# PoTaTo-Mika/fish-speech

Hardware: AMD Instinct MI355X
Metric: audio-sec/wall-sec (RTF) + p50 first-sample latency, S2-Pro 4B @1/2/4/8 GPU (higher is better)
Workload: dtype bf16; 1 GPU; BASELINE config 2 per GPU: one utterance = 64-token prompt + 216 Dual-AR frames (top_k 30, top_p 0.8, temp 0.8) + codec decode [1,10,216] -> 442368 samples; global_batch=1, frames=216, prompt_len=64, first_chunk_frames=1, vocoder_chunks=first_chunk_frames, then growing 4x, vocoder=serial, parallelism=dp1

## Files before the change

fish-speech_amd/csrc/fm_attn.hip:

```cpp
#include "fm_kernels.h"
#include "fm_runtime.h"
#include "fm_attn_dev.h"
#include "fm_frag.h"

template <typename T>
__device__ __forceinline__ void head_prep(const T* src, int hd, bool norm, const T* nw, float eps,
                                          const float* tab, bool do_rope, float (&x0)[2],
                                          float (&x1)[2], int& np, int lane) {
    const int half = hd >> 1;
    np = 0;
    for (int p = lane; p < half; p += 64, ++np) {
        x0[np] = ld(src, 2 * p);
        x1[np] = ld(src, 2 * p + 1);
    }
    if (norm) {
        float ss = 0.f;
        for (int i = 0; i < np; ++i) ss += x0[i] * x0[i] + x1[i] * x1[i];
        ss = wave_sum(ss);
        const float rs = 1.0f / sqrtf(ss / (float)hd + eps);
        for (int i = 0; i < np; ++i) {
            const int p = lane + 64 * i;
            x0[i] = rnd<T>((x0[i] * rs) * ld(nw, 2 * p));
            x1[i] = rnd<T>((x1[i] * rs) * ld(nw, 2 * p + 1));
        }
// ... 491 lines not shown
}
template <typename T> __device__ __forceinline__ typename Frag<T>::f frag_f32(const float* v) {
    typename Frag<T>::f f;
    if constexpr (sizeof(T) == 2) {
#pragma unroll
        for (int i = 0; i < 4; ++i) f[i] = hi_pair(v[2 * i], v[2 * i + 1]);
    } else {
#pragma unroll
        for (int i = 0; i < 4; ++i) {
            f.lo[i] = v[i];
            f.hi[i] = v[4 + i];
        }
    }
    return f;
}
template <typename T, int HD, int NW>
__global__ __launch_bounds__(NW * 64) void attn_fd_kernel(AttnDecArgs<T> a) {
    static_assert(HD % 32 == 0 && HD <= 128, "head_dim a multiple of 32 up to 128");
    constexpr int NT = NW * 64, FD_TILE = 16 * NW;
    constexpr int VL = 8 * (int)sizeof(T) / 16;
    constexpr int half = HD / 2;
    __shared__ __attribute__((aligned(16))) float q_s[FD_GM][HD];
    __shared__ __attribute__((aligned(16))) float kv_new[2][HD];
    __shared__ __attribute__((aligned(16))) float wml[NW][FD_GM][2];
    constexpr int OG = NW > 4 ? 1 : 4;
    __shared__ __attribute__((aligned(16))) float ored[NW][OG][FD_GM][HD];
    __shared__ int flag;
    unsigned long long tz[7] = {0, 0, 0, 0, 0, 0, 0};
    DBG_TS(tz, 0)
    const int lane = threadIdx.x & 63, wave = threadIdx.x >> 6;
    const int l16 = lane & 15, qq = lane >> 4;
    const int r = blockIdx.x, kvh = blockIdx.y, sp = blockIdx.z;
    const int g = a.nh / a.nkv, nitem = g + 2;
    const int slot = a.row_slot[r];
    const int pos = a.row_pos[r];
    constexpr int NI = (2 + FD_GM + NW - 1) / NW;
    float x0[NI], x1[NI];
#pragma unroll
    for (int i = 0; i < NI; ++i) {
        const int it = wave + NW * i;
        const int row = it < g ? kvh * g + it : (it == g ? a.nh + kvh : a.nh + a.nkv + kvh);
        const bool ok = it < nitem && lane < half;
        float v0, v1;
        raw_pair<T>(a.qkv, a.ldqkv, a.qslab, a.qslab_kp, gridDim.x, a.qbias, r,
                    (size_t)(it < nitem ? row : 0) * HD + 2 * (lane < half ? lane : 0), v0, v1);
        x0[i] = ok ? v0 : 0.f;
        x1[i] = ok ? v1 : 0.f;
    }
    const int npos = pos + 1;
    int nsp = min((int)gridDim.z, (npos + a.cap - 1) / a.cap);
    const int chunk = ((npos + nsp - 1) / nsp + 15) & ~15;
    nsp = (npos + chunk - 1) / chunk;
    if (sp >= nsp) return;
    const int j0 = sp * chunk, jend = min(j0 + chunk, npos);
    const bool owner = jend == npos;
    const size_t base = (size_t)slot * a.slot_stride + a.layer_off + (size_t)kvh * a.S * HD;
    T* kc = a.kc + base;
    T* vc = a.vc + base;
    const int vd = 8 * l16 < HD ? 8 * l16 : HD - 8;
    using F = Frag<T>;
    constexpr int NKS = HD / 32;
    typename F::f kb[NKS];
    u32x4_t vb[4][VL];
    auto issue = [&](int jb) {
        const int jk = min(jb + 16 * wave + l16, jend - 1);
// ... 23 lines not shown
                x0[i] = rnd<T>((x0[i] * rs) * ld(nw, 2 * lane));
                x1[i] = rnd<T>((x1[i] * rs) * ld(nw, 2 * lane + 1));
            }
        }
        if (lane < half) {
            float y0 = x0[i], y1 = x1[i];
            if (isq || isk) {
                const float c = rcs.x, sn = rcs.y;
                y0 = rnd<T>(x0[i] * c - x1[i] * sn);
                y1 = rnd<T>(x1[i] * c + x0[i] * sn);
            }
            if (isq) {
                q_s[it][2 * lane] = y0;
                q_s[it][2 * lane + 1] = y1;
                if (a.qdbg && sp == 0) {
                    float* qdp = a.qdbg + ((size_t)r * a.nh + kvh * g + it) * HD;
                    qdp[2 * lane] = y0;
                    qdp[2 * lane + 1] = y1;
                }
            } else {
                kv_new[isk ? 0 : 1][2 * lane] = y0;
                kv_new[isk ? 0 : 1][2 * lane + 1] = y1;
                T* dst = (isk ? kc : vc) + (size_t)pos * HD;
                st(dst, 2 * lane, y0);
                st(dst, 2 * lane + 1, y1);
            }
        }
    }
    lds_barrier();
    DBG_TS(tz, 1)
    const int qh = l16 >> 2;
    const bool qrow = (l16 & 3) == 0 && qh < g;
    typename F::f qa[NKS];
#pragma unroll
    for (int ks = 0; ks < NKS; ++ks) {
        float qv[8];
#pragma unroll
        for (int e = 0; e < 8; ++e) qv[e] = qrow ? q_s[qh][32 * ks + 8 * qq + e] : 0.f;
        qa[ks] = frag_f32<T>(qv);
    }
    __shared__ __attribute__((aligned(16))) float p_s[NW][16][FD_GM];
    float m_run = -INFINITY, l_run = 0.f, o[FD_GM][8];
#pragma unroll
    for (int h = 0; h < FD_GM; ++h)
#pragma unroll
        for (int e = 0; e < 8; ++e) o[h][e] = 0.f;
    const int npass = (jend - j0 + FD_TILE - 1) / FD_TILE;
    for (int pa = 0; pa < npass; ++pa) {
        const int jb = j0 + pa * FD_TILE;
        const int jk = jb + 16 * wave + l16;
        if (owner && jk == pos) {
#pragma unroll
            for (int ks = 0; ks < NKS; ++ks) kb[ks] = frag_f32<T>(&kv_new[0][32 * ks + 8 * qq]);
        }
        f32x4_t sc = {0.f, 0.f, 0.f, 0.f};
#pragma unroll
        for (int ks = 0; ks < NKS; ++ks) sc = F::mma(qa[ks], kb[ks], sc);
        float vf[4][8];
#pragma unroll
// ... 9 lines not shown
        if (owner) {
#pragma unroll
            for (int it = 0; it < 4; ++it)
                if (min(jb + 16 * wave + 4 * it + qq, jend - 1) == pos)
#pragma unroll
                    for (int e = 0; e < 8; ++e) vf[it][e] = kv_new[1][vd + e];
        }
        const bool kval = jk < jend && qq < g;
        {
            const float sv = kval ? sc[0] * a.scale : -INFINITY;
            const float mnew = fmaxf(m_run, row_max16(sv));
            const float alpha = mnew == -INFINITY ? 1.f : expf(m_run - mnew);
            const float p = kval ? expf(sv - mnew) : 0.f;
            m_run = mnew;
            l_run = l_run * alpha + p;
            p_s[wave][l16][qq] = p;
#pragma unroll
            for (int h = 0; h < FD_GM; ++h) {
                if (h >= g) break;
                const float ah = __int_as_float(__builtin_amdgcn_readlane(__float_as_int(alpha), 16 * h));
#pragma unroll
                for (int e = 0; e < 8; ++e) o[h][e] *= ah;
            }
        }
        __builtin_amdgcn_wave_barrier();
#pragma unroll
        for (int it = 0; it < 4; ++it) {
            const f32x4_t pv = *reinterpret_cast<const f32x4_t*>(&p_s[wave][4 * it + qq][0]);
#pragma unroll
            for (int h = 0; h < FD_GM; ++h) {
                if (h >= g) break;
#pragma unroll
                for (int e = 0; e < 8; ++e) o[h][e] += pv[h] * vf[it][e];
            }
        }
        __builtin_amdgcn_wave_barrier();
    }
    DBG_TS(tz, 2)
    const float lrow = row_sum16(l_run);
    if (l16 == 0 && qq < g) {
        wml[wave][qq][0] = m_run;
        wml[wave][qq][1] = lrow;
    }
#pragma unroll
    for (int h = 0; h < FD_GM; ++h) {
        if (h >= g) break;
        if constexpr (OG == 1) {
#pragma unroll
            for (int e = 0; e < 8; ++e) o[h][e] = sum_rows4(o[h][e], lane);
        }
        if (8 * l16 < HD && (OG == 4 || qq == 0)) {
            f32x4_t* dst = reinterpret_cast<f32x4_t*>(&ored[wave][OG == 4 ? qq : 0][h][8 * l16]);
            dst[0] = (f32x4_t){o[h][0], o[h][1], o[h][2], o[h][3]};
            dst[1] = (f32x4_t){o[h][4], o[h][5], o[h][6], o[h][7]};
        }
    }
    DBG_TS(tz, 5)
    lds_barrier();
    DBG_TS(tz, 3)
    const bool single = nsp == 1;
// ... 1 lines not shown
        const int h = idx / HD, e = idx - h * HD;
        float M = wml[0][h][0];
#pragma unroll
        for (int w = 1; w < NW; ++w) M = fmaxf(M, wml[w][h][0]);
        float L = 0.f, O = 0.f;
#pragma unroll
        for (int w = 0; w < NW; ++w) {
            const float sc = expf(wml[w][h][0] - M);
            L += sc * wml[w][h][1];
            if constexpr (OG == 4)
                O += sc * ((ored[w][0][h][e] + ored[w][1][h][e]) + (ored[w][2][h][e] + ored[w][3][h][e]));
            else
                O += sc * ored[w][0][h][e];
        }
        if (single) {
            st(a.out + (size_t)r * a.nh * HD + (size_t)(kvh * g + h) * HD, e, O / L);
        } else {
            float* pp = a.part + (((size_t)r * a.nh + (size_t)kvh * g + h) * a.maxsplit + sp) * (HD + 2);
            __hip_atomic_store(pp + 2 + e, O, __ATOMIC_RELAXED, __HIP_MEMORY_SCOPE_AGENT);
            if (e == 0) {
                __hip_atomic_store(pp, M, __ATOMIC_RELAXED, __HIP_MEMORY_SCOPE_AGENT);
                __hip_atomic_store(pp + 1, L, __ATOMIC_RELAXED, __HIP_MEMORY_SCOPE_AGENT);
            }
        }
    }
    if (a.dbg && threadIdx.x == 0) {
        tz[4] = __builtin_amdgcn_s_memrealtime();
        dbg_record(a.dbg, 0xFFFC, (unsigned)(nsp << 16 | (jend - j0)), tz);
    }
    if (single) return;
    asm volatile("s_waitcnt vmcnt(0)" ::: "memory");
    __syncthreads();
    if (threadIdx.x == 0) {
        const int t = __hip_atomic_fetch_add(a.cnt + (size_t)r * a.nkv + kvh, 1, __ATOMIC_RELAXED,
                                             __HIP_MEMORY_SCOPE_AGENT);
        flag = t == nsp - 1;
        if (t == nsp - 1) __hip_atomic_store(a.cnt + (size_t)r * a.nkv + kvh, 0, __ATOMIC_RELAXED, __HIP_MEMORY_SCOPE_AGENT);
    }
    __syncthreads();
    if (!flag) return;
    DBG_TS(tz, 5)
    constexpr int PP = FD_GM * HD * 8 / NT;
    const int q = l16, grp = threadIdx.x >> 4;
    const int k0 = grp * PP, h = k0 / half, e0 = 2 * (k0 - h * half);
    if (h >= g) return;
    const int qc = q < nsp ? q : nsp - 1;
    const unsigned long long* pp = reinterpret_cast<const unsigned long long*>(
        a.part + (((size_t)r * a.nh + (size_t)kvh * g + h) * a.maxsplit + qc) * (HD + 2));
    const unsigned long long ml = __hip_atomic_load(pp, __ATOMIC_RELAXED, __HIP_MEMORY_SCOPE_AGENT);
    unsigned long long ov[PP];
#pragma unroll
    for (int j = 0; j < PP; ++j) ov[j] = __hip_atomic_load(pp + 1 + e0 / 2 + j, __ATOMIC_RELAXED, __HIP_MEMORY_SCOPE_AGENT);
    const float mq = q < nsp ? __uint_as_float((unsigned)ml) : -INFINITY;
    const float lq = __uint_as_float((unsigned)(ml >> 32));
    float M = mq;
#pragma unroll
    for (int m = 1; m < 16; m <<= 1) M = fmaxf(M, __shfl_xor(M, m));
    const float w = q < nsp ? expf(mq - M) : 0.f;
    float L = w * lq;
#pragma unroll
    for (int m = 1; m < 16; m <<= 1) L += __shfl_xor(L, m);
    T* out = a.out + (size_t)r * a.nh * HD + (size_t)(kvh * g + h) * HD + e0;
#pragma unroll
    for (int j = 0; j < PP; ++j) {
        float o0 = w * __uint_as_float((unsigned)ov[j]), o1 = w * __uint_as_float((unsigned)(ov[j] >> 32));
#pragma unroll
        for (int m = 1; m < 16; m <<= 1) {
            o0 += __shfl_xor(o0, m);
            o1 += __shfl_xor(o1, m);
        }
        if (q == (j & 15)) {
            st(out, 2 * j, o0 / L);
            st(out, 2 * j + 1, o1 / L);
        }
    }
    if (a.dbg && threadIdx.x == 0) {
        tz[6] = __builtin_amdgcn_s_memrealtime();
// ... 750 lines not shown
                                      : ((code >= 0 && code < a.cb) ? code : 0);
    }
    record();
}

template <typename T> void launch_attn_decode2(hipStream_t s, const AttnDecArgs<T>& a, int R) {
    dim3 g1(R, a.nkv, a.maxsplit);
    static bool attr = false;
    if (!attr) {
        (void)hipFuncSetAttribute(reinterpret_cast<const void*>(&attn_decode2_kernel<T>),
                                  hipFuncAttributeMaxDynamicSharedMemorySize, 160 * 1024);
        attr = true;
    }
    attn_decode2_kernel<T><<<g1, 512, attn2_lds_bytes(a.hd, a.nh / a.nkv, a.cap, sizeof(T)), s>>>(a);
}
template <typename T> void launch_attn_fd(hipStream_t s, const AttnDecArgs<T>& a0, int R) {
    FMCHECK(attn_fd_ok(a0.hd, a0.nh / a0.nkv), "attn_fd: head_dim 32, 64 or 128 and at most 4 q heads per kv head");
    FMCHECK(a0.cap >= 16 && a0.cnt && a0.part && a0.out, "attn_fd: min split >= 16, tickets, partials and output set");
    AttnDecArgs<T> a = a0;
    a.maxsplit = std::min(FD_NSP, FM_CEIL(a.S, a.cap));
    const dim3 grid(R, a.nkv, a.maxsplit);
    if (a.nwb == 16) {
        switch (a.hd) {
            case 32: attn_fd_kernel<T, 32, 16><<<grid, 1024, 0, s>>>(a); break;
            case 64: attn_fd_kernel<T, 64, 16><<<grid, 1024, 0, s>>>(a); break;
            default: attn_fd_kernel<T, 128, 16><<<grid, 1024, 0, s>>>(a); break;
        }
        return;
    }
    if (a.nwb == 8) {
        switch (a.hd) {
            case 32: attn_fd_kernel<T, 32, 8><<<grid, 512, 0, s>>>(a); break;
            case 64: attn_fd_kernel<T, 64, 8><<<grid, 512, 0, s>>>(a); break;
            default: attn_fd_kernel<T, 128, 8><<<grid, 512, 0, s>>>(a); break;
        }
        return;
    }
    switch (a.hd) {
        case 32: attn_fd_kernel<T, 32, 4><<<grid, 256, 0, s>>>(a); break;
        case 64: attn_fd_kernel<T, 64, 4><<<grid, 256, 0, s>>>(a); break;
        default: attn_fd_kernel<T, 128, 4><<<grid, 256, 0, s>>>(a); break;
    }
}
template <typename T> void launch_attn_decode3(hipStream_t s, const AttnDecArgs<T>& a0, int R) {
    FMCHECK(a0.hd % 32 == 0 && a0.hd <= 128 && a0.nh % a0.nkv == 0 && a0.nh / a0.nkv <= 6,
            "attn_dec3: hd a multiple of 32 up to 128, at most 6 q heads per kv head");
    AttnDecArgs<T> a = a0;
    a.maxsplit = FM_CEIL(a.S, ATT3_CH);
    attn_dec3_kernel<T><<<dim3(R, a.nkv, a.maxsplit), 256, 0, s>>>(a);
}
template <typename T> void launch_fast_attn2(hipStream_t s, const FastFusedArgs<T>& a, int R) {
    fast_attn2_kernel<T><<<dim3(R, a.nh), 64, 0, s>>>(a);
}
template <typename T> void launch_fast_attn_fused(hipStream_t s, const FastFusedArgs<T>& a, int R) {
    dim3 g(R, a.nkv);
    const size_t lds = (size_t)2 * a.S * a.hd * 4 + (size_t)4 * a.hd * 4 + 4 * 64 * 4;
    fast_attn_fused_kernel<T><<<g, 256, lds, s>>>(a);
// ... 33 lines not shown
```

fish-speech_amd/csrc/fm_kernels.h:

```cpp
#pragma once
#include <algorithm>
#include "fm_common.h"
#include "fm_tune_table.h"

enum { EPI_STORE = 0, EPI_RESID = 1, EPI_SWIGLU = 2, EPI_F32 = 3 };

template <typename T> void launch_swiglu_i8(hipStream_t s, const T* t, int ldt, T* act, int lda, int inter, int R);
template <typename T> void launch_pack(hipStream_t s, const T* src, int N, int K, T* dst);
template <typename T> void launch_quant_rows(hipStream_t s, T* w, int N, int K, int8_t* q, T* scale);
template <typename T> void launch_i8_to(hipStream_t s, const int8_t* q, int64_t n, T* dst);
void launch_pack_q8(hipStream_t s, const int8_t* src, int N, int K, int8_t* dst);
void launch_pack_q8s(hipStream_t s, const int8_t* src, int N, int K, int8_t* dst);
void launch_quant4(hipStream_t s, bf16_t* w, int N, int K, int gs, uint8_t* q, uint32_t* sz);
void launch_pack_q4(hipStream_t s, const uint8_t* q, int N, int K, uint8_t* dst);
void launch_pack_q4_rows(hipStream_t s, const uint8_t* q, int N, int K, uint32_t* dst);
void launch_pack_sz4(hipStream_t s, const uint32_t* sz, int N, int K, int gs, uint32_t* dst);
void launch_pack_q4s(hipStream_t s, const uint8_t* q, int N, int K, uint32_t* dst);

template <typename T> struct LinearArgs {
    const T* W;
    const T* W2;
    const T* bias;
    const T* X;
    int ldx, R, N, K;
// ... 359 lines not shown
    const T* qn;
    const T* kn;
    const float* rope;
    T* kc;
    T* vc;
    size_t slot_stride, layer_off;
    int S, maxsplit;
    float scale;
    float* part;
    int cap;
    int* cnt;
    T* out;
    unsigned long long* dbg;
    float* qdbg = nullptr;
    int nwb = 4;
    const float* qslab = nullptr;
    int qslab_kp = 1;
    const T* qbias = nullptr;
};
template <typename T> void launch_attn_decode2(hipStream_t s, const AttnDecArgs<T>& a, int R);
inline size_t attn2_lds_bytes(int hd, int g, int cap, size_t esz) {
    return (size_t)cap * (hd + 8) * esz + (size_t)cap * hd * esz + (size_t)g * hd * 4 + (size_t)g * cap * 4 +
           16 + 8 * (size_t)g * 4;
}
inline int attn2_cap(int hd, int g, size_t esz) {
    long budget = 150L * 1024 - 16 - 8L * g * 4 - (long)g * hd * 4;
    long per = (long)(2 * hd + 8) * (long)esz + 4L * g;
    long c = budget / per;
    c = c > 256 ? 256 : c;
    return (int)(c & ~15L);
// ... 14 lines not shown
```

fish-speech_amd/csrc/fm_llm_frame.cpp:

```cpp
#include <math.h>

#include <algorithm>
#include <array>

#include "fm_codec.h"
#include "fm_llm_model.h"

template <typename T> struct Run {
    typedef T type_t;
    fm_llm* m;
    hipStream_t s;
    int64_t E;
    bool rows_distinct_slots = false, bs_frame = false, x_ss = false;
    struct BsPending {
        bool on = false;
        const float* slab = nullptr;
        int kparts = 0, d = 0, R = 0;
        void* res = nullptr;
        void* out = nullptr;
        const void* sc = nullptr;
    } pend;
    std::vector<std::array<int, 2>> segs;
    void set_pending(const float* slab, int kparts, int d, int R, void* res, void* out, const void* sc) {
        pend = BsPending{true, slab, kparts, d, R, res, out, sc};
// ... 159 lines not shown
        const int64_t bytes = step_wbytes(a.Wq4s ? 2 : (a.Wq8s ? 1 : 0), N, K, E) + (int64_t)R * K * E +
                              (int64_t)R * N * (epi == EPI_F32 ? 4 : E);
        const double flops = 2.0 * R * N * K;
        hipStream_t st = s;
        auto go = [st, a, epi] { launch_linear<T>(st, a, epi); };
        launch(cls, bytes, flops, go);
    }

    void attn_slow(const AttnDecArgs<T>& aa, int R) { attn_slow_on(s, aa, R); }
    static void attn_slow_on(hipStream_t s, const AttnDecArgs<T>& aa, int R) {
        const AttnSlowPlan p = attn_slow_plan(R, aa.hd, aa.nh / aa.nkv, aa.cap);
        if (p.kernel == 3) {
            AttnDecArgs<T> b = aa;
            b.cap = p.cap;
            b.nwb = p.nwb;
            launch_attn_fd<T>(s, b, R);
        } else if (p.kernel == 2)
            launch_attn_decode3<T>(s, aa, R);
        else
            launch_attn_decode2<T>(s, aa, R);
    }
    bool bs_use(int R, bool) const {
        return (fm_tuning().bstream || m->compact) && bs_frame && R > GEMV_MAX_ROWS && R <= 32 && m->bsA;
    }
    struct BsExtra {
        int pro = PRO_PLAIN;
        const float* ss_in = nullptr;
        const void* nw = nullptr;
        const void* res = nullptr;
        void* res_out = nullptr;
// ... 1281 lines not shown
```

fish-speech_amd/csrc/fm_llm_model.h:

```cpp
#pragma once
#include <hip/hip_runtime.h>

#include <algorithm>

#include "fm_kernels.h"
#include "fm_runtime.h"

static constexpr int PREFILL_CHUNK = 1024;
static constexpr int ATTN_PIECE = 256;
static constexpr int ATTN_SPLIT = 64;
static constexpr int GEMV_MAX_ROWS = 8;
static constexpr int KSB_MAX = 8;

inline int attn2_frame_cap(int hd, int g, size_t esz, bool batched) {
    const int cap = attn2_cap(hd, g, esz), knob = batched ? fm_tuning().attn_cap_batched : fm_tuning().attn_cap;
    return knob ? std::min(cap, knob) : cap;
}
struct AttnSlowPlan {
    int kernel, nwb, cap;
};
inline AttnSlowPlan attn_slow_plan(int R, int hd, int g, int cap0) {
    const FmTuning& tu = fm_tuning();
    if (tu.attn_fd && attn_fd_ok(hd, g)) {
        AttnSlowPlan p{3, 4, std::max(16, R > GEMV_MAX_ROWS ? tu.fd_min_batched : tu.fd_min)};
        if (R <= GEMV_MAX_ROWS && tu.fd_nw > 4) {
            p.nwb = tu.fd_nw;
            p.cap = std::max(16, tu.fd_min16);
        } else if (R > GEMV_MAX_ROWS && tu.fd_nw_batched > 4) {
            p.nwb = tu.fd_nw_batched;
        }
        return p;
    }
    if (tu.attn3 && R > GEMV_MAX_ROWS && hd % 32 == 0 && hd <= 128 && g <= 6) return {2, 4, cap0};
    return {0, 4, cap0};
}
static constexpr int BS_KPARTS = 8;

inline int pick_ksb(int N, int K, int R, size_t esz) {
    const int nb = (N + 15) / 16;
// ... 174 lines not shown
```

fish-speech_amd/csrc/fm_llm_weights.cpp:

```cpp
#include "fm_llm_model.h"

void add_t(fm_llm* m, const std::string& n, int64_t rows, int64_t cols) {
    DTensor t;
    t.rows = rows;
    t.cols = cols;
    t.numel = rows * cols;
    m->w[n] = t;
}
static void add_stack(fm_llm* m, const std::string& pre, const StackDims& s) {
    for (int i = 0; i < s.n_layer; ++i) {
        std::string p = pre + std::to_string(i) + ".";
        add_t(m, p + "attention.wqkv.weight", s.nqkv(), s.dim);
        if (s.qkv_bias) add_t(m, p + "attention.wqkv.bias", 1, s.nqkv());
        add_t(m, p + "attention.wo.weight", s.dim, s.nq());
        if (s.o_bias) add_t(m, p + "attention.wo.bias", 1, s.dim);
        if (s.qk_norm) {
            add_t(m, p + "attention.q_norm.weight", 1, s.hd);
            add_t(m, p + "attention.k_norm.weight", 1, s.hd);
        }
        add_t(m, p + "feed_forward.w1.weight", s.inter, s.dim);
        add_t(m, p + "feed_forward.w3.weight", s.inter, s.dim);
        add_t(m, p + "feed_forward.w2.weight", s.dim, s.inter);
        add_t(m, p + "ffn_norm.weight", 1, s.dim);
        add_t(m, p + "attention_norm.weight", 1, s.dim);
// ... 432 lines not shown
    m->xl = m->dalloc((size_t)n * dmax * E);
    m->plast = m->dalloc((size_t)n * dmax * E);
    m->xnl = m->dalloc((size_t)n * dmax * E);
    m->fx = m->dalloc((size_t)std::max(n, 2) * dmax * E);
    m->fh = m->dalloc((size_t)std::max(n, 2) * dmax * E);
    m->fxn = m->dalloc((size_t)n * dmax * E);
    m->x2 = m->dalloc((size_t)std::min(n, GEMV_MAX_ROWS) * dmax * E);
    m->fx2 = m->dalloc((size_t)std::max(std::min(n, GEMV_MAX_ROWS), 2) * dmax * E);
    m->chain_cnt = (unsigned*)m->dalloc(GEMV_CHAIN_WORDS * sizeof(unsigned));
    m->chain_err = (int*)m->dalloc(16 * sizeof(int));
    HIPCHK(hipHostMalloc((void**)&m->h_chain_err, 16 * sizeof(int), hipHostMallocDefault));
    m->h_chain_err[0] = 0;
    m->maxsplit = FM_CEIL(m->S, ATTN_SPLIT);
    const int Rpart = std::max(m->max_slots, ATTN_PIECE);
    m->part = (float*)m->dalloc((size_t)Rpart * d.nh * std::max(m->maxsplit, FM_CEIL(m->S, 16)) * (d.hd + 2) * 4, false);
    m->attn_cnt = (int*)m->dalloc((size_t)R * d.nkv * sizeof(int));
    m->ssX = (float*)m->dalloc((size_t)(dmax / 16) * std::min(n, 32) * 4);
    m->ssH = (float*)m->dalloc((size_t)(dmax / 16) * std::min(n, 32) * 4);
    {
        const int maxn = std::max({m->Nhead, 2 * c.intermediate_size, 2 * c.fast_intermediate_size, qkvmax, dmax, m->cb});
        m->tickets = (int*)m->dalloc((size_t)(maxn / 16 + 16) * sizeof(int));
        m->fin_cnt = (int*)m->dalloc((size_t)std::max(m->max_slots, 64) * 2 * sizeof(int));
        m->fin_ss = (float*)m->dalloc((size_t)std::max(m->max_slots, 64) * 16 * sizeof(float));
        m->skpart_cap = 16ll << 20;
        m->skpart = (float*)m->dalloc((size_t)m->skpart_cap * sizeof(float), false);
    }
    HIPCHK(hipMemsetAsync(m->attn_cnt, 0, (size_t)R * d.nkv * sizeof(int), m->stream));
    m->slabA = (float*)m->dalloc((size_t)KSB_MAX * std::min(n, GEMV_MAX_ROWS) * dmax * 4);
    m->slabB = (float*)m->dalloc((size_t)KSB_MAX * std::min(n, GEMV_MAX_ROWS) * dmax * 4);
    if (n > GEMV_MAX_ROWS) {
        m->bsA = (float*)m->dalloc((size_t)BS_KPARTS * 32 * dmax * 4, false);
        m->bsB = (float*)m->dalloc((size_t)BS_KPARTS * 32 * dmax * 4, false);
        m->bsQ = (float*)m->dalloc((size_t)BS_KPARTS * 32 * std::max(m->sd.nqkv(), m->fdm.nqkv()) * 4, false);
    }
    m->logits = (float*)m->dalloc((size_t)n * m->Nhead * 4);
    m->flogits = (float*)m->dalloc((size_t)n * m->cb * 4);
    m->frame_slot = (int*)m->dalloc(n * 4);
    m->frame_pos = (int*)m->dalloc(n * 4);
    m->prow_slot = (int*)m->dalloc(PREFILL_CHUNK * 4);
    m->prow_pos = (int*)m->dalloc(PREFILL_CHUNK * 4);
    m->pfx_slots = (int*)m->dalloc((size_t)n * 4);
    m->tok_in = (int32_t*)m->dalloc((size_t)n * m->C1 * 4);
// ... 15 lines not shown
```

fish-speech_amd/csrc/fm_ops.cpp:

```cpp
#include <hip/hip_runtime.h>
#include <math.h>
#include <string.h>

#include <algorithm>
#include <vector>

#include "fm_codec.h"
#include "fm_kernels.h"
#include "fm_llm_model.h"
#include "fm_ops_util.h"
#include "fm_runtime.h"

using namespace fm_ops_util;

namespace {

struct TuneScope {
    int& knob;
    const int keep;
    TuneScope(int& k, int v) : knob(k), keep(k) { knob = v; }
    ~TuneScope() { knob = keep; }
};

template <typename T>
// ... 72 lines not shown
    const size_t stride = (size_t)nkv * S * hd;
    T* kc = (T*)b.alloc(stride * sizeof(T));
    T* vc = (T*)b.alloc(stride * sizeof(T));
    T* out = (T*)b.alloc((size_t)nh * hd * sizeof(T));
    float* qd = (float*)b.alloc((size_t)nh * hd * 4);
    int* row = (int*)b.alloc(8);
    const int rs[2] = {0, pos};
    b.put(row, rs, 8);
    const float scale = 1.0f / sqrtf((float)hd);
    if (kernel == 0 || kernel == 2 || kernel == 3) {
        AttnDecArgs<T> a{raw, ld, row, row + 1, nh, nkv, hd, qk_norm, eps, qnd, knd, rope, kc, vc, stride, 0, S,
                         1, scale, nullptr};
        a.cap = attn2_cap(hd, nh / nkv, sizeof(T));
        a.maxsplit = FM_CEIL(S, std::min(a.cap, 16));
        a.part = (float*)b.alloc((size_t)nh * a.maxsplit * (hd + 2) * 4);
        a.cnt = (int*)b.alloc((size_t)nkv * 4);
        a.out = out;
        a.qdbg = qd;
        if (kernel == 2) {
            launch_attn_decode3<T>(s, a, 1);
        } else if (kernel == 3) {
            FMCHECK(attn_fd_ok(hd, nh / nkv), "attn_fd: head_dim 32, 64 or 128, at most 4 q heads per kv head");
            a.cap = std::max(16, fm_tuning().fd_min16);
            a.nwb = fm_tuning().fd_nw;
            a.maxsplit = FM_CEIL(S, a.cap);
            launch_attn_fd<T>(s, a, 1);
        } else {
            a.maxsplit = FM_CEIL(S, a.cap);
            launch_attn_decode2<T>(s, a, 1);
        }
    } else {
        FMCHECK(pos < 16, "fast attention positions are < 16");
        FastFusedArgs<T> a{raw, ld, row, nh, nkv, hd, qk_norm, eps, qnd, knd, rope, kc, vc, stride, 0, S, pos,
                           scale, out};
        a.qdbg = qd;
        launch_fast_attn2<T>(s, a, 1);
    }
    HIPCHK(hipGetLastError());
    HIPCHK(hipMemcpyAsync(q_out, qd, (size_t)nh * hd * 4, hipMemcpyDeviceToHost, s));
// ... 42 lines not shown
    T* kc = b.upload<T>(kcache, (size_t)R * stride);
    T* vc = b.upload<T>(vcache, (size_t)R * stride);
    T* o = (T*)b.alloc((size_t)R * nh * hd * sizeof(T));
    int* rows = (int*)b.alloc((size_t)2 * R * 4);
    std::vector<int> rs(2 * R);
    for (int r = 0; r < R; ++r) {
        rs[r] = r;
        rs[R + r] = pos[r];
    }
    b.put(rows, rs.data(), rs.size() * 4);
    AttnDecArgs<T> a{raw, ld, rows, rows + R, nh, nkv, hd, qk_norm, eps, qnd, knd, rope, kc, vc, stride, 0, S,
                     1, 1.0f / sqrtf((float)hd), nullptr};
    const int g = nh / nkv;
    a.maxsplit = FM_CEIL(S, 16);
    a.part = (float*)b.alloc((size_t)R * nh * a.maxsplit * (hd + 2) * 4);
    a.cnt = (int*)b.alloc((size_t)R * nkv * 4);
    a.out = o;
    if (kernel == 3) {
        FMCHECK(attn_fd_ok(hd, g), "attn_fd: head_dim 32, 64 or 128 and at most 4 q heads per kv head");
        a.cap = min_split;
        launch_attn_fd<T>(s, a, R);
    } else if (kernel == 2) {
        FMCHECK(hd % 32 == 0 && hd <= 128 && g <= 6, "attn_dec3: hd a multiple of 32 up to 128, g <= 6");
        launch_attn_decode3<T>(s, a, R);
    } else {
        a.cap = std::min(min_split, attn2_cap(hd, g, sizeof(T)));
        a.maxsplit = FM_CEIL(S, a.cap);
        launch_attn_decode2<T>(s, a, R);
    }
    HIPCHK(hipGetLastError());
    download<T>(o, (size_t)R * nh * hd, out, s);
    download<T>(kc, (size_t)R * stride, kc_out, s);
    download<T>(vc, (size_t)R * stride, vc_out, s);
}

// ... 37 lines not shown
    const T* raw = o.qkv ? b.upload<T>(o.qkv, (size_t)R * ld) : nullptr;
    const float* slab = o.slab ? upload_raw(b, o.slab, (size_t)o.kp * R * ld) : nullptr;
    const T* bias = o.bias ? b.upload<T>(o.bias, (size_t)ld) : nullptr;
    T* qnd = o.qk_norm ? b.upload<T>(o.qn, (size_t)hd) : (T*)b.alloc((size_t)hd * sizeof(T));
    T* knd = o.qk_norm ? b.upload<T>(o.kn, (size_t)hd) : (T*)b.alloc((size_t)hd * sizeof(T));
    float* rope = upload_rope(b, S, hd, o.base);
    const size_t layer_stride = (size_t)nkv * S * hd, slot_stride = (size_t)o.layers * layer_stride;
    InOut<T> kc(b, o.kc, (size_t)o.nslots * slot_stride), vc(b, o.vc, (size_t)o.nslots * slot_stride);
    T* out = (T*)b.alloc((size_t)R * nh * hd * sizeof(T));
    std::vector<int> rs(2 * R);
    for (int r = 0; r < R; ++r) {
        rs[r] = o.row_slot[r];
        rs[R + r] = o.pos[r];
    }
    int* rows = upload_i32(b, rs.data(), rs.size());
    int kernel = o.kernel, nwb = o.nwb, cap = o.cap;
    const int cap2 = attn2_cap(hd, g, sizeof(T));
    if (o.frame) {
        const AttnSlowPlan p = attn_slow_plan(R, hd, g, attn2_frame_cap(hd, g, sizeof(T), R > GEMV_MAX_ROWS));
        kernel = p.kernel;
        nwb = p.nwb;
        cap = p.cap;
    }
    if (kernel == 0) cap = std::min(cap, cap2);
    FMCHECK(!slab || kernel == 3, "the slab form of the QKV input needs attn_fd");
    FMCHECK(kernel != 3 || attn_fd_ok(hd, g), "attn_fd: head_dim 32, 64 or 128 and at most 4 q heads per kv head");
    FMCHECK(kernel != 2 || (hd % 32 == 0 && hd <= 128 && g <= 6), "attn_dec3: hd a multiple of 32 up to 128, g <= 6");
    const int maxsplit = kernel == 3 ? std::min(FD_NSP, FM_CEIL(S, cap)) : (kernel == 2 ? FM_CEIL(S, 64) : FM_CEIL(S, cap));
    AttnDecArgs<T> a{raw, ld, rows, rows + R, nh, nkv, hd, o.qk_norm, o.eps, qnd, knd, rope, kc.d, vc.d, slot_stride,
                     (size_t)o.layer * layer_stride, S, maxsplit, 1.0f / sqrtf((float)hd), nullptr};
    const size_t npart = (size_t)R * nh * maxsplit * (hd + 2);
    a.part = (float*)b.alloc((npart + PART_GUARD) * 4);
    HIPCHK(hipMemsetAsync(a.part, 0xff, npart * 4, s));
    const std::vector<uint32_t> guard(PART_GUARD, 0x5a5a5a5au);
    b.put(a.part + npart, guard.data(), PART_GUARD * 4);
    a.cnt = (int*)b.alloc((size_t)R * nkv * 4);
    a.out = out;
    a.cap = cap;
    a.nwb = nwb;
    a.qslab = slab;
    a.qslab_kp = o.kp;
    a.qbias = bias;
    for (int i = 0; i < o.reps; ++i) {
        if (kernel == 3)
            launch_attn_fd<T>(s, a, R);
        else if (kernel == 2)
            launch_attn_decode3<T>(s, a, R);
        else
            launch_attn_decode2<T>(s, a, R);
        HIPCHK(hipGetLastError());
    }
    download<T>(out, (size_t)R * nh * hd, o.out, s);
    kc.get(s);
    vc.get(s);
    std::vector<uint32_t> back(PART_GUARD);
    HIPCHK(hipMemcpyAsync(back.data(), a.part + npart, PART_GUARD * 4, hipMemcpyDeviceToHost, s));
    HIPCHK(hipStreamSynchronize(s));
    const int info[8] = {kernel, nwb, cap, maxsplit, count_nonzero(a.cnt, (size_t)R * nkv, s), back == guard, FD_NSP, cap2};
    memcpy(o.info, info, sizeof(info));
}

struct SlotRows {
    const int *row_slot, *row_pos;
    int nslots, layers, layer;
};
template <typename T>
void qk_rope_cache_t(hipStream_t s, const float* qkv, const float* slabh, int kp, const float* biash, int R, int nh,
                     int nkv, int hd, const float* qn, const float* kn, int qk_norm, float eps, float base,
                     const SlotRows& sr, int fixed_pos, float* kch, float* vch, int S, float* q_out) {
    DevBufs b(s);
    const int ld = (nh + 2 * nkv) * hd;
    const T* raw = qkv ? b.upload<T>(qkv, (size_t)R * ld) : nullptr;
    const float* slab = slabh ? upload_raw(b, slabh, (size_t)kp * R * ld) : nullptr;
// ... 1644 lines not shown
```

fish-speech_amd/csrc/fm_tune_table.h:

```cpp
#ifndef FM_TUNE_RULES
#define FM_TUNE_RULES
enum { FM_RULE_BOOL, FM_RULE_ANY, FM_RULE_SET, FM_RULE_RANGE, FM_RULE_MULT16 };
template <typename... V> constexpr int fm_knob_set(V... v) { return (0 | ... | (1 << v)); }
#define FM_BOOL FM_RULE_BOOL, 0, 0
#define FM_ANY FM_RULE_ANY, 0, 0
#define FM_SET(...) FM_RULE_SET, fm_knob_set(__VA_ARGS__), 0
#define FM_RANGE(lo, hi) FM_RULE_RANGE, lo, hi
#define FM_MIN(lo) FM_RULE_RANGE, lo, 0x7fffffff
#define FM_MULT16 FM_RULE_MULT16, 0, 0
#define FM_ZERO_OR_MULT16 FM_RULE_MULT16, 1, 0
#endif

#ifdef FM_KNOB
FM_KNOB(gemv_nt, 1, FM_BOOL)
FM_KNOB(gemv_u, 8, FM_SET(2, 4, 8))
FM_KNOB(gemv_wpb, 4, FM_SET(4, 8))
FM_KNOB(sampler_kth, 1, FM_BOOL)
FM_KNOB(sampler_fast, 1, FM_BOOL)
FM_KNOB(attn_cap, 32, FM_ZERO_OR_MULT16)
FM_KNOB(attn_wo, 0, FM_BOOL)
FM_KNOB(ksb_blocks, 512, FM_MIN(1))
FM_KNOB(batched_fused_attn, 1, FM_BOOL)
FM_KNOB(attn_cap_batched, 128, FM_ZERO_OR_MULT16)
FM_KNOB(linear_u32, 4, FM_SET(4, 8))
FM_KNOB(linear_fill, 0, FM_MIN(0))
FM_KNOB(attn3, 1, FM_BOOL)
FM_KNOB(attn_fd, 1, FM_BOOL)
FM_KNOB(fd_min, 32, FM_MULT16)
FM_KNOB(fd_min_batched, 512, FM_MULT16)
FM_KNOB(fd_nw, 8, FM_SET(4, 8, 16))
FM_KNOB(fin_ksb, 0, FM_RANGE(0, 8))
FM_KNOB(fd_nw_batched, 4, FM_SET(4, 8, 16))
FM_KNOB(fd_min16, 256, FM_MULT16)
FM_KNOB(prefill_attn, 1, FM_BOOL)
FM_KNOB(prompt_gemm, 1, FM_BOOL)
FM_KNOB(prompt_skinny, 1, FM_BOOL)
FM_KNOB(prompt_skinny_blocks, 256, FM_MIN(1))
FM_KNOB(prompt_unroll, 1, FM_BOOL)
FM_KNOB(prompt_qkv_slab, 1, FM_BOOL)
FM_KNOB(prompt_fin, 1, FM_BOOL)
FM_KNOB(prompt_swiglu, 1, FM_BOOL)
FM_KNOB(prompt_skinny_q, 1, FM_RANGE(0, 2))
FM_KNOB(prompt_gemm_q, 1, FM_RANGE(0, 2))
FM_KNOB(prompt_ks_tiles, 384, FM_MIN(1))
FM_KNOB(prompt_ks_max, 8, FM_SET(1, 2, 4, 8))
FM_KNOB(conv2, 1, FM_BOOL)
FM_KNOB(conv_splitk, 1, FM_BOOL)
FM_KNOB(resunit_cfg, 1, FM_RANGE(0, 2))
// ... 45 lines not shown
```

Measured before the change: 12.12 audio-sec/wall-sec.

## Split flash-decode attention blocks across query-head groups for small batches

Adds a GM template parameter to the flash-decode attention kernel so each block handles 1, 2 or all query heads of a KV head. The head groups are folded into the z grid dimension to launch more blocks at low batch. The goal is better occupancy and lower latency in single-row decode. The cost is that each KV-cache tile is read once per head group instead of once per KV head, which adds memory traffic and duplicates the q/k norm and rope work. Only group 0 writes the new KV entry, and the ticket counters are resized to one per q head. A new knob fd_hpb defaults to 1 head per block for small row counts.

```diff
diff --git a/fish-speech_amd/csrc/fm_attn.hip b/fish-speech_amd/csrc/fm_attn.hip
--- a/fish-speech_amd/csrc/fm_attn.hip
+++ b/fish-speech_amd/csrc/fm_attn.hip
@@ -529,32 +529,34 @@
     }
     return f;
 }
-template <typename T, int HD, int NW>
+template <typename T, int HD, int NW, int GM>
 __global__ __launch_bounds__(NW * 64) void attn_fd_kernel(AttnDecArgs<T> a) {
+    static_assert(GM == 1 || GM == 2 || GM == FD_GM, "1, 2 or every q head of the kv head");
     static_assert(HD % 32 == 0 && HD <= 128, "head_dim a multiple of 32 up to 128");
     constexpr int NT = NW * 64, FD_TILE = 16 * NW;
     constexpr int VL = 8 * (int)sizeof(T) / 16;
     constexpr int half = HD / 2;
-    __shared__ __attribute__((aligned(16))) float q_s[FD_GM][HD];
+    __shared__ __attribute__((aligned(16))) float q_s[GM][HD];
     __shared__ __attribute__((aligned(16))) float kv_new[2][HD];
-    __shared__ __attribute__((aligned(16))) float wml[NW][FD_GM][2];
+    __shared__ __attribute__((aligned(16))) float wml[NW][GM][2];
     constexpr int OG = NW > 4 ? 1 : 4;
-    __shared__ __attribute__((aligned(16))) float ored[NW][OG][FD_GM][HD];
+    __shared__ __attribute__((aligned(16))) float ored[NW][OG][GM][HD];
     __shared__ int flag;
     unsigned long long tz[7] = {0, 0, 0, 0, 0, 0, 0};
     DBG_TS(tz, 0)
     const int lane = threadIdx.x & 63, wave = threadIdx.x >> 6;
     const int l16 = lane & 15, qq = lane >> 4;
-    const int r = blockIdx.x, kvh = blockIdx.y, sp = blockIdx.z;
-    const int g = a.nh / a.nkv, nitem = g + 2;
+    const int r = blockIdx.x, kvh = blockIdx.y;
+    const int hg = GM == FD_GM ? 0 : (int)blockIdx.z / a.maxsplit, sp = (int)blockIdx.z - hg * a.maxsplit;
+    const int g = min(GM, a.nh / a.nkv - hg * GM), h0 = kvh * (a.nh / a.nkv) + hg * GM, nitem = g + 2;
     const int slot = a.row_slot[r];
     const int pos = a.row_pos[r];
-    constexpr int NI = (2 + FD_GM + NW - 1) / NW;
+    constexpr int NI = (2 + GM + NW - 1) / NW;
     float x0[NI], x1[NI];
 #pragma unroll
     for (int i = 0; i < NI; ++i) {
         const int it = wave + NW * i;
-        const int row = it < g ? kvh * g + it : (it == g ? a.nh + kvh : a.nh + a.nkv + kvh);
+        const int row = it < g ? h0 + it : (it == g ? a.nh + kvh : a.nh + a.nkv + kvh);
         const bool ok = it < nitem && lane < half;
         float v0, v1;
         raw_pair<T>(a.qkv, a.ldqkv, a.qslab, a.qslab_kp, gridDim.x, a.qbias, r,
@@ -563,7 +565,7 @@
         x1[i] = ok ? v1 : 0.f;
     }
     const int npos = pos + 1;
-    int nsp = min((int)gridDim.z, (npos + a.cap - 1) / a.cap);
+    int nsp = min(a.maxsplit, (npos + a.cap - 1) / a.cap);
     const int chunk = ((npos + nsp - 1) / nsp + 15) & ~15;
     nsp = (npos + chunk - 1) / chunk;
     if (sp >= nsp) return;
@@ -617,16 +619,18 @@
                 q_s[it][2 * lane] = y0;
                 q_s[it][2 * lane + 1] = y1;
                 if (a.qdbg && sp == 0) {
-                    float* qdp = a.qdbg + ((size_t)r * a.nh + kvh * g + it) * HD;
+                    float* qdp = a.qdbg + ((size_t)r * a.nh + h0 + it) * HD;
                     qdp[2 * lane] = y0;
                     qdp[2 * lane + 1] = y1;
                 }
             } else {
                 kv_new[isk ? 0 : 1][2 * lane] = y0;
                 kv_new[isk ? 0 : 1][2 * lane + 1] = y1;
-                T* dst = (isk ? kc : vc) + (size_t)pos * HD;
-                st(dst, 2 * lane, y0);
-                st(dst, 2 * lane + 1, y1);
+                if (hg == 0) {
+                    T* dst = (isk ? kc : vc) + (size_t)pos * HD;
+                    st(dst, 2 * lane, y0);
+                    st(dst, 2 * lane + 1, y1);
+                }
             }
         }
     }
@@ -639,13 +643,13 @@
     for (int ks = 0; ks < NKS; ++ks) {
         float qv[8];
 #pragma unroll
-        for (int e = 0; e < 8; ++e) qv[e] = qrow ? q_s[qh][32 * ks + 8 * qq + e] : 0.f;
+        for (int e = 0; e < 8; ++e) qv[e] = qrow ? q_s[qh < GM ? qh : 0][32 * ks + 8 * qq + e] : 0.f;
         qa[ks] = frag_f32<T>(qv);
     }
-    __shared__ __attribute__((aligned(16))) float p_s[NW][16][FD_GM];
-    float m_run = -INFINITY, l_run = 0.f, o[FD_GM][8];
-#pragma unroll
-    for (int h = 0; h < FD_GM; ++h)
+    __shared__ __attribute__((aligned(16))) float p_s[NW][16][GM];
+    float m_run = -INFINITY, l_run = 0.f, o[GM][8];
+#pragma unroll
+    for (int h = 0; h < GM; ++h)
 #pragma unroll
         for (int e = 0; e < 8; ++e) o[h][e] = 0.f;
     const int npass = (jend - j0 + FD_TILE - 1) / FD_TILE;
@@ -685,9 +689,9 @@
             const float p = kval ? expf(sv - mnew) : 0.f;
             m_run = mnew;
             l_run = l_run * alpha + p;
-            p_s[wave][l16][qq] = p;
-#pragma unroll
-            for (int h = 0; h < FD_GM; ++h) {
+            if (GM == FD_GM || qq < GM) p_s[wave][l16][qq] = p;
+#pragma unroll
+            for (int h = 0; h < GM; ++h) {
                 if (h >= g) break;
                 const float ah = __int_as_float(__builtin_amdgcn_readlane(__float_as_int(alpha), 16 * h));
 #pragma unroll
@@ -697,9 +701,18 @@
         __builtin_amdgcn_wave_barrier();
 #pragma unroll
         for (int it = 0; it < 4; ++it) {
-            const f32x4_t pv = *reinterpret_cast<const f32x4_t*>(&p_s[wave][4 * it + qq][0]);
-#pragma unroll
-            for (int h = 0; h < FD_GM; ++h) {
+            float pv[GM];
+            if constexpr (GM == 4) {
+                const f32x4_t t = *reinterpret_cast<const f32x4_t*>(&p_s[wave][4 * it + qq][0]);
+                pv[0] = t[0], pv[1] = t[1], pv[2] = t[2], pv[3] = t[3];
+            } else if constexpr (GM == 2) {
+                const float2 t = *reinterpret_cast<const float2*>(&p_s[wave][4 * it + qq][0]);
+                pv[0] = t.x, pv[1] = t.y;
+            } else {
+                pv[0] = p_s[wave][4 * it + qq][0];
+            }
+#pragma unroll
+            for (int h = 0; h < GM; ++h) {
                 if (h >= g) break;
 #pragma unroll
                 for (int e = 0; e < 8; ++e) o[h][e] += pv[h] * vf[it][e];
@@ -708,13 +721,15 @@
         __builtin_amdgcn_wave_barrier();
     }
     DBG_TS(tz, 2)
+    __shared__ unsigned long long wend[NW];
+    if (a.dbg && lane == 0) wend[wave] = __builtin_amdgcn_s_memrealtime();
     const float lrow = row_sum16(l_run);
     if (l16 == 0 && qq < g) {
         wml[wave][qq][0] = m_run;
         wml[wave][qq][1] = lrow;
     }
 #pragma unroll
-    for (int h = 0; h < FD_GM; ++h) {
+    for (int h = 0; h < GM; ++h) {
         if (h >= g) break;
         if constexpr (OG == 1) {
 #pragma unroll
@@ -746,9 +761,9 @@
                 O += sc * ored[w][0][h][e];
         }
         if (single) {
-            st(a.out + (size_t)r * a.nh * HD + (size_t)(kvh * g + h) * HD, e, O / L);
+            st(a.out + (size_t)r * a.nh * HD + (size_t)(h0 + h) * HD, e, O / L);
         } else {
-            float* pp = a.part + (((size_t)r * a.nh + (size_t)kvh * g + h) * a.maxsplit + sp) * (HD + 2);
+            float* pp = a.part + (((size_t)r * a.nh + h0 + h) * a.maxsplit + sp) * (HD + 2);
             __hip_atomic_store(pp + 2 + e, O, __ATOMIC_RELAXED, __HIP_MEMORY_SCOPE_AGENT);
             if (e == 0) {
                 __hip_atomic_store(pp, M, __ATOMIC_RELAXED, __HIP_MEMORY_SCOPE_AGENT);
@@ -758,27 +773,28 @@
     }
     if (a.dbg && threadIdx.x == 0) {
         tz[4] = __builtin_amdgcn_s_memrealtime();
+        for (int w = 0; w < NW; ++w) tz[6] = wend[w] > tz[6] ? wend[w] : tz[6];
         dbg_record(a.dbg, 0xFFFC, (unsigned)(nsp << 16 | (jend - j0)), tz);
     }
     if (single) return;
     asm volatile("s_waitcnt vmcnt(0)" ::: "memory");
     __syncthreads();
     if (threadIdx.x == 0) {
-        const int t = __hip_atomic_fetch_add(a.cnt + (size_t)r * a.nkv + kvh, 1, __ATOMIC_RELAXED,
-                                             __HIP_MEMORY_SCOPE_AGENT);
+        int* tk = a.cnt + (size_t)r * a.nh + kvh * (a.nh / a.nkv) + hg;
+        const int t = __hip_atomic_fetch_add(tk, 1, __ATOMIC_RELAXED, __HIP_MEMORY_SCOPE_AGENT);
         flag = t == nsp - 1;
-        if (t == nsp - 1) __hip_atomic_store(a.cnt + (size_t)r * a.nkv + kvh, 0, __ATOMIC_RELAXED, __HIP_MEMORY_SCOPE_AGENT);
+        if (t == nsp - 1) __hip_atomic_store(tk, 0, __ATOMIC_RELAXED, __HIP_MEMORY_SCOPE_AGENT);
     }
     __syncthreads();
     if (!flag) return;
     DBG_TS(tz, 5)
-    constexpr int PP = FD_GM * HD * 8 / NT;
+    constexpr int PP = GM * HD * 8 / NT > 0 ? GM * HD * 8 / NT : 1;
     const int q = l16, grp = threadIdx.x >> 4;
     const int k0 = grp * PP, h = k0 / half, e0 = 2 * (k0 - h * half);
     if (h >= g) return;
     const int qc = q < nsp ? q : nsp - 1;
     const unsigned long long* pp = reinterpret_cast<const unsigned long long*>(
-        a.part + (((size_t)r * a.nh + (size_t)kvh * g + h) * a.maxsplit + qc) * (HD + 2));
+        a.part + (((size_t)r * a.nh + h0 + h) * a.maxsplit + qc) * (HD + 2));
     const unsigned long long ml = __hip_atomic_load(pp, __ATOMIC_RELAXED, __HIP_MEMORY_SCOPE_AGENT);
     unsigned long long ov[PP];
 #pragma unroll
@@ -792,7 +808,7 @@
     float L = w * lq;
 #pragma unroll
     for (int m = 1; m < 16; m <<= 1) L += __shfl_xor(L, m);
-    T* out = a.out + (size_t)r * a.nh * HD + (size_t)(kvh * g + h) * HD + e0;
+    T* out = a.out + (size_t)r * a.nh * HD + (size_t)(h0 + h) * HD + e0;
 #pragma unroll
     for (int j = 0; j < PP; ++j) {
         float o0 = w * __uint_as_float((unsigned)ov[j]), o1 = w * __uint_as_float((unsigned)(ov[j] >> 32));
@@ -1573,33 +1589,33 @@
     }
     attn_decode2_kernel<T><<<g1, 512, attn2_lds_bytes(a.hd, a.nh / a.nkv, a.cap, sizeof(T)), s>>>(a);
 }
+template <typename T, int NW, int GM> static void attn_fd_go(hipStream_t s, const AttnDecArgs<T>& a, int R) {
+    const dim3 grid(R, a.nkv, a.maxsplit * FM_CEIL(a.nh / a.nkv, GM));
+    switch (a.hd) {
+        case 32: attn_fd_kernel<T, 32, NW, GM><<<grid, NW * 64, 0, s>>>(a); break;
+        case 64: attn_fd_kernel<T, 64, NW, GM><<<grid, NW * 64, 0, s>>>(a); break;
+        default: attn_fd_kernel<T, 128, NW, GM><<<grid, NW * 64, 0, s>>>(a); break;
+    }
+}
+template <typename T, int NW> static void attn_fd_hpb(hipStream_t s, const AttnDecArgs<T>& a, int R) {
+    switch (a.hpb) {
+        case 1: attn_fd_go<T, NW, 1>(s, a, R); break;
+        case 2: attn_fd_go<T, NW, 2>(s, a, R); break;
+        default: attn_fd_go<T, NW, FD_GM>(s, a, R); break;
+    }
+}
 template <typename T> void launch_attn_fd(hipStream_t s, const AttnDecArgs<T>& a0, int R) {
     FMCHECK(attn_fd_ok(a0.hd, a0.nh / a0.nkv), "attn_fd: head_dim 32, 64 or 128 and at most 4 q heads per kv head");
     FMCHECK(a0.cap >= 16 && a0.cnt && a0.part && a0.out, "attn_fd: min split >= 16, tickets, partials and output set");
+    FMCHECK(a0.hpb == 1 || a0.hpb == 2 || a0.hpb == FD_GM, "attn_fd: 1, 2 or 4 q heads per block");
     AttnDecArgs<T> a = a0;
     a.maxsplit = std::min(FD_NSP, FM_CEIL(a.S, a.cap));
-    const dim3 grid(R, a.nkv, a.maxsplit);
-    if (a.nwb == 16) {
-        switch (a.hd) {
-            case 32: attn_fd_kernel<T, 32, 16><<<grid, 1024, 0, s>>>(a); break;
-            case 64: attn_fd_kernel<T, 64, 16><<<grid, 1024, 0, s>>>(a); break;
-            default: attn_fd_kernel<T, 128, 16><<<grid, 1024, 0, s>>>(a); break;
-        }
-        return;
-    }
-    if (a.nwb == 8) {
-        switch (a.hd) {
-            case 32: attn_fd_kernel<T, 32, 8><<<grid, 512, 0, s>>>(a); break;
-            case 64: attn_fd_kernel<T, 64, 8><<<grid, 512, 0, s>>>(a); break;
-            default: attn_fd_kernel<T, 128, 8><<<grid, 512, 0, s>>>(a); break;
-        }
-        return;
-    }
-    switch (a.hd) {
-        case 32: attn_fd_kernel<T, 32, 4><<<grid, 256, 0, s>>>(a); break;
-        case 64: attn_fd_kernel<T, 64, 4><<<grid, 256, 0, s>>>(a); break;
-        default: attn_fd_kernel<T, 128, 4><<<grid, 256, 0, s>>>(a); break;
-    }
+    if (a.nwb == 16)
+        attn_fd_hpb<T, 16>(s, a, R);
+    else if (a.nwb == 8)
+        attn_fd_hpb<T, 8>(s, a, R);
+    else
+        attn_fd_hpb<T, 4>(s, a, R);
 }
 template <typename T> void launch_attn_decode3(hipStream_t s, const AttnDecArgs<T>& a0, int R) {
     FMCHECK(a0.hd % 32 == 0 && a0.hd <= 128 && a0.nh % a0.nkv == 0 && a0.nh / a0.nkv <= 6,
diff --git a/fish-speech_amd/csrc/fm_kernels.h b/fish-speech_amd/csrc/fm_kernels.h
--- a/fish-speech_amd/csrc/fm_kernels.h
+++ b/fish-speech_amd/csrc/fm_kernels.h
@@ -397,6 +397,7 @@
     unsigned long long* dbg;
     float* qdbg = nullptr;
     int nwb = 4;
+    int hpb = 4;
     const float* qslab = nullptr;
     int qslab_kp = 1;
     const T* qbias = nullptr;
diff --git a/fish-speech_amd/csrc/fm_llm_frame.cpp b/fish-speech_amd/csrc/fm_llm_frame.cpp
--- a/fish-speech_amd/csrc/fm_llm_frame.cpp
+++ b/fish-speech_amd/csrc/fm_llm_frame.cpp
@@ -197,6 +197,7 @@
             AttnDecArgs<T> b = aa;
             b.cap = p.cap;
             b.nwb = p.nwb;
+            b.hpb = p.hpb;
             launch_attn_fd<T>(s, b, R);
         } else if (p.kernel == 2)
             launch_attn_decode3<T>(s, aa, R);
diff --git a/fish-speech_amd/csrc/fm_llm_model.h b/fish-speech_amd/csrc/fm_llm_model.h
--- a/fish-speech_amd/csrc/fm_llm_model.h
+++ b/fish-speech_amd/csrc/fm_llm_model.h
@@ -18,11 +18,13 @@
 }
 struct AttnSlowPlan {
     int kernel, nwb, cap;
-};
+    int hpb = 4;
+};
+inline int fd_hpb_rows(int R) { return R <= GEMV_MAX_ROWS ? fm_tuning().fd_hpb : 4; }
 inline AttnSlowPlan attn_slow_plan(int R, int hd, int g, int cap0) {
     const FmTuning& tu = fm_tuning();
     if (tu.attn_fd && attn_fd_ok(hd, g)) {
-        AttnSlowPlan p{3, 4, std::max(16, R > GEMV_MAX_ROWS ? tu.fd_min_batched : tu.fd_min)};
+        AttnSlowPlan p{3, 4, std::max(16, R > GEMV_MAX_ROWS ? tu.fd_min_batched : tu.fd_min), fd_hpb_rows(R)};
         if (R <= GEMV_MAX_ROWS && tu.fd_nw > 4) {
             p.nwb = tu.fd_nw;
             p.cap = std::max(16, tu.fd_min16);
diff --git a/fish-speech_amd/csrc/fm_llm_weights.cpp b/fish-speech_amd/csrc/fm_llm_weights.cpp
--- a/fish-speech_amd/csrc/fm_llm_weights.cpp
+++ b/fish-speech_amd/csrc/fm_llm_weights.cpp
@@ -470,7 +470,8 @@
     m->maxsplit = FM_CEIL(m->S, ATTN_SPLIT);
     const int Rpart = std::max(m->max_slots, ATTN_PIECE);
     m->part = (float*)m->dalloc((size_t)Rpart * d.nh * std::max(m->maxsplit, FM_CEIL(m->S, 16)) * (d.hd + 2) * 4, false);
-    m->attn_cnt = (int*)m->dalloc((size_t)R * d.nkv * sizeof(int));
+    const size_t ncnt = std::max((size_t)R * d.nkv, (size_t)m->max_slots * d.nh);
+    m->attn_cnt = (int*)m->dalloc(ncnt * sizeof(int));
     m->ssX = (float*)m->dalloc((size_t)(dmax / 16) * std::min(n, 32) * 4);
     m->ssH = (float*)m->dalloc((size_t)(dmax / 16) * std::min(n, 32) * 4);
     {
@@ -481,7 +482,7 @@
         m->skpart_cap = 16ll << 20;
         m->skpart = (float*)m->dalloc((size_t)m->skpart_cap * sizeof(float), false);
     }
-    HIPCHK(hipMemsetAsync(m->attn_cnt, 0, (size_t)R * d.nkv * sizeof(int), m->stream));
+    HIPCHK(hipMemsetAsync(m->attn_cnt, 0, ncnt * sizeof(int), m->stream));
     m->slabA = (float*)m->dalloc((size_t)KSB_MAX * std::min(n, GEMV_MAX_ROWS) * dmax * 4);
     m->slabB = (float*)m->dalloc((size_t)KSB_MAX * std::min(n, GEMV_MAX_ROWS) * dmax * 4);
     if (n > GEMV_MAX_ROWS) {
diff --git a/fish-speech_amd/csrc/fm_ops.cpp b/fish-speech_amd/csrc/fm_ops.cpp
--- a/fish-speech_amd/csrc/fm_ops.cpp
+++ b/fish-speech_amd/csrc/fm_ops.cpp
@@ -110,7 +110,7 @@
         a.cap = attn2_cap(hd, nh / nkv, sizeof(T));
         a.maxsplit = FM_CEIL(S, std::min(a.cap, 16));
         a.part = (float*)b.alloc((size_t)nh * a.maxsplit * (hd + 2) * 4);
-        a.cnt = (int*)b.alloc((size_t)nkv * 4);
+        a.cnt = (int*)b.alloc((size_t)nh * 4);
         a.out = out;
         a.qdbg = qd;
         if (kernel == 2) {
@@ -119,6 +119,7 @@
             FMCHECK(attn_fd_ok(hd, nh / nkv), "attn_fd: head_dim 32, 64 or 128, at most 4 q heads per kv head");
             a.cap = std::max(16, fm_tuning().fd_min16);
             a.nwb = fm_tuning().fd_nw;
+            a.hpb = fd_hpb_rows(1);
             a.maxsplit = FM_CEIL(S, a.cap);
             launch_attn_fd<T>(s, a, 1);
         } else {
@@ -191,11 +192,12 @@
     const int g = nh / nkv;
     a.maxsplit = FM_CEIL(S, 16);
     a.part = (float*)b.alloc((size_t)R * nh * a.maxsplit * (hd + 2) * 4);
-    a.cnt = (int*)b.alloc((size_t)R * nkv * 4);
+    a.cnt = (int*)b.alloc((size_t)R * nh * 4);
     a.out = o;
     if (kernel == 3) {
         FMCHECK(attn_fd_ok(hd, g), "attn_fd: head_dim 32, 64 or 128 and at most 4 q heads per kv head");
         a.cap = min_split;
+        a.hpb = fd_hpb_rows(R);
         launch_attn_fd<T>(s, a, R);
     } else if (kernel == 2) {
         FMCHECK(hd % 32 == 0 && hd <= 128 && g <= 6, "attn_dec3: hd a multiple of 32 up to 128, g <= 6");
@@ -263,13 +265,14 @@
         rs[R + r] = o.pos[r];
     }
     int* rows = upload_i32(b, rs.data(), rs.size());
-    int kernel = o.kernel, nwb = o.nwb, cap = o.cap;
+    int kernel = o.kernel, nwb = o.nwb, cap = o.cap, hpb = fd_hpb_rows(R);
     const int cap2 = attn2_cap(hd, g, sizeof(T));
     if (o.frame) {
         const AttnSlowPlan p = attn_slow_plan(R, hd, g, attn2_frame_cap(hd, g, sizeof(T), R > GEMV_MAX_ROWS));
         kernel = p.kernel;
         nwb = p.nwb;
         cap = p.cap;
+        hpb = p.hpb;
     }
     if (kernel == 0) cap = std::min(cap, cap2);
     FMCHECK(!slab || kernel == 3, "the slab form of the QKV input needs attn_fd");
@@ -283,10 +286,11 @@
     HIPCHK(hipMemsetAsync(a.part, 0xff, npart * 4, s));
     const std::vector<uint32_t> guard(PART_GUARD, 0x5a5a5a5au);
     b.put(a.part + npart, guard.data(), PART_GUARD * 4);
-    a.cnt = (int*)b.alloc((size_t)R * nkv * 4);
+    a.cnt = (int*)b.alloc((size_t)R * nh * 4);
     a.out = out;
     a.cap = cap;
     a.nwb = nwb;
+    a.hpb = hpb;
     a.qslab = slab;
     a.qslab_kp = o.kp;
     a.qbias = bias;
@@ -305,7 +309,7 @@
     std::vector<uint32_t> back(PART_GUARD);
     HIPCHK(hipMemcpyAsync(back.data(), a.part + npart, PART_GUARD * 4, hipMemcpyDeviceToHost, s));
     HIPCHK(hipStreamSynchronize(s));
-    const int info[8] = {kernel, nwb, cap, maxsplit, count_nonzero(a.cnt, (size_t)R * nkv, s), back == guard, FD_NSP, cap2};
+    const int info[8] = {kernel, nwb, cap, maxsplit, count_nonzero(a.cnt, (size_t)R * nh, s), back == guard, FD_NSP, cap2};
     memcpy(o.info, info, sizeof(info));
 }
 
diff --git a/fish-speech_amd/csrc/fm_tune_table.h b/fish-speech_amd/csrc/fm_tune_table.h
--- a/fish-speech_amd/csrc/fm_tune_table.h
+++ b/fish-speech_amd/csrc/fm_tune_table.h
@@ -32,6 +32,7 @@
 FM_KNOB(fin_ksb, 0, FM_RANGE(0, 8))
 FM_KNOB(fd_nw_batched, 4, FM_SET(4, 8, 16))
 FM_KNOB(fd_min16, 256, FM_MULT16)
+FM_KNOB(fd_hpb, 1, FM_SET(1, 2, 4))
 FM_KNOB(prefill_attn, 1, FM_BOOL)
 FM_KNOB(prompt_gemm, 1, FM_BOOL)
 FM_KNOB(prompt_skinny, 1, FM_BOOL)
```

After: 12.48 audio-sec/wall-sec, median of 6. 3.0% higher.
